# writingindy/SWMHD

Hardware: AMD Instinct MI355X
Metric: Mcell-steps/sec (fp64) on 4096^2 periodic grid (higher is better)
Workload: dtype f64

## Files before the change

swmhd_amd/csrc/common.hpp:

```cpp
#pragma once
#include <hip/hip_runtime.h>
#include <stdint.h>
#include <stdio.h>
#include <stdlib.h>
#include <type_traits>

namespace swmhd {

template <typename T>
struct OpArgs {
    const T *A;
    const T *h;
    T *Fx;
    T *Fy;
    int Nx, Ny, Hx, Hy;
    long sy;
    T dx, dy, rdx, rdy;
    int j0, j1;
    int topo_x, topo_y;
    int kernel_variant;
    int edge_cols;
};

template <typename T> hipError_t launch_lorentz_jacobian_fast(const OpArgs<T> &a, hipStream_t s);
template <typename T> hipError_t launch_lorentz_jacobian_strict(const OpArgs<T> &a, hipStream_t s);
template <typename T> hipError_t launch_lorentz_divergence_fast(const OpArgs<T> &a, hipStream_t s);
template <typename T> hipError_t launch_lorentz_divergence_strict(const OpArgs<T> &a, hipStream_t s);

template <typename T>
hipError_t launch_fill_halo_periodic(T *interior, int Nx, int Ny, int Hx, int Hy, long sy, int which, hipStream_t s);
template <typename T>
hipError_t launch_fill_halo_periodic_multi(T *const *interiors, int nfields, int Nx, int Ny, int Hx, int Hy, long sy,
                                           int which, hipStream_t s, int members = 0, long stride_m = 0);
template <typename T>
struct HaloBc {
    T *f[4];
    T grad[4][4];
    int nf, Nx, Ny, Hx, Hy, topo_x, topo_y, face_x, face_y;
    long sy;
    T dx, dy;
};
template <typename T> hipError_t launch_fill_halo_bc(const HaloBc<T> &a, hipStream_t s);
template <typename T>
struct HaloBcEns : HaloBc<T> {
    long stride_m;
    int members;
    const T *gtab;
};
template <typename T> hipError_t launch_fill_halo_bc_ensemble(const HaloBcEns<T> &a, hipStream_t s);

template <typename T>
struct TendArgs {
    const T *q1, *q2, *h, *A;
    T *G1, *G2, *Gh, *GA;
    int Nx, Ny, Hx, Hy;
    long sy;
    T dx, dy, rdx, rdy, grav, fcor;
    int j0, j1;
    int j0b, j1b;
    int fuse, first, store_G;
    int gm_prev;
    int drop_G;
    int wrap;
    int kernel_variant;
    int topo_x, topo_y;
    int leave_room;
    int edge_cols;
    T *Unew[4];
    const T *Gm[4];
    T dt, gamma, zeta;
    T dtg;
    T cu, cg;
    int anchor;
    T dtw;
};
template <typename T>
struct EnsTendArgs : TendArgs<T> {
    long stride_m;
    int members;
    int fold;
};
template <typename T, bool ENS> using TileArgs = std::conditional_t<ENS, EnsTendArgs<T>, TendArgs<T>>;
constexpr int GM_IS_PREV_STATE = 1024;
constexpr int RK3_ANCHOR = 2048;
constexpr double RK3_ANCHOR_WEIGHT = 0.25;
template <typename T>
struct Rk3Stage {
    T gamma, zeta;
    int store_G;
    const T *const *Gm;
    int flags;
};
template <typename T>
struct Rk3Buffers {
    T *cur[4], *alt[4], *gn[4], *gm[4];
    int swaps = 0;
    bool set(T *const *q, T *const *q_alt, T *const *Ga, T *const *Gb) {
        for (int f = 0; f < 4; ++f) {
            if (!q[f] || !q_alt[f] || !Ga[f] || !Gb[f]) return false;
            cur[f] = q[f]; alt[f] = q_alt[f]; gn[f] = Ga[f]; gm[f] = Gb[f];
        }
        return true;
    }
    Rk3Stage<T> stage(int st, bool anchor) const {
        const T gam[3] = {T(8.0 / 15.0), T(5.0 / 12.0), T(3.0 / 4.0)};
        const T zet[3] = {T(0), T(-17.0 / 60.0), T(-5.0 / 12.0)};
        if (anchor) return {gam[st], st == 0 ? T(RK3_ANCHOR_WEIGHT) : T(0), 0, st == 0 ? nullptr : (st == 1 ? gm : gn), RK3_ANCHOR};
        return {gam[st], zet[st], st < 2 ? 1 : 0, st == 0 ? nullptr : gm, 0};
    }
    void rotate() {
        for (int f = 0; f < 4; ++f) { T *t = cur[f]; cur[f] = alt[f]; alt[f] = t; t = gn[f]; gn[f] = gm[f]; gm[f] = t; }
        ++swaps;
    }
};

template <typename T>
struct Rk3Args {
    T *U[4];
    const T *Gn[4];
    const T *Gm[4];
    int Nx;
    long sy;
    int j0, j1;
    T dt, gamma, zeta;
    int first;
};
typedef int sw_v2i __attribute__((ext_vector_type(2)));
typedef float sw_f2 __attribute__((ext_vector_type(2)));
typedef sw_f2 sw_f2_u __attribute__((aligned(4)));
constexpr unsigned SW_OOB = 0xFFFFFFC0u;
template <typename T> __device__ __forceinline__ __amdgpu_buffer_rsrc_t out_rsrc(T *parent, unsigned bytes) {
    return __builtin_amdgcn_make_buffer_rsrc(parent, 0, (int)bytes, 0x00020000);
}
template <typename T> __device__ __forceinline__ void buffer_store(T v, __amdgpu_buffer_rsrc_t r, unsigned off) {
    if constexpr (sizeof(T) == 8) __builtin_amdgcn_raw_buffer_store_b64(__builtin_bit_cast(sw_v2i, v), r, off, 0, 0);
    else __builtin_amdgcn_raw_buffer_store_b32(__builtin_bit_cast(int, v), r, off, 0, 0);
}
template <int N> __device__ __forceinline__ void wait_vmem_all_but() {
    static_assert(N >= 0 && N < 64, "vmcnt is a 6-bit counter");
    __builtin_amdgcn_s_waitcnt((N & 15) | ((N >> 4) << 14) | (7 << 4) | (15 << 8));
}

struct ProgressPriority {
    int t1, t2, t3;
    __device__ __forceinline__ explicit ProgressPriority(int niter)
        : t1((niter * 3) / 5), t2((niter * 17) / 20), t3((niter * 19) / 20) {
        __builtin_amdgcn_s_setprio(3);
    }
    __device__ __forceinline__ void at(int it) const {
        if (it == t1) __builtin_amdgcn_s_setprio(2);
        if (it == t2) __builtin_amdgcn_s_setprio(1);
        if (it == t3) __builtin_amdgcn_s_setprio(0);
    }
};

struct MarchGeometry {
    int nt;
    int nstrips, nseg, LY;
    int wg_per_cu;
};
inline int device_cu_count() {
    static int cus = 0;
    if (cus <= 0) {
        int dev = 0, n = 0;
        if (hipGetDevice(&dev) != hipSuccess || hipDeviceGetAttribute(&n, hipDeviceAttributeMultiprocessorCount, dev) != hipSuccess || n <= 0)
            n = 256;
        cus = n;
    }
    return cus;
}
inline int env_knob(const char *name, int &cache) {
    if (cache == 0) {
        const char *e = getenv(name);
        const int v = e ? atoi(e) : 0;
        cache = v > 0 ? v : -1;
    }
    return cache > 0 ? cache : 0;
}
inline int leave_room_64ths(int rows) {
    static int cache = 0;
    const int v = env_knob("SWMHD_RING_ROOM", cache);
    return v > 0 ? (v < 32 ? v : 32) : (rows >= 3072 ? 1 : 3);
}
inline MarchGeometry march_geometry(int Nx, int rows, int xh, const int *nts, const int *wgs, int ncand, int ly_min, bool leave_room,
                                    int force_nt, int force_ly) {
    MarchGeometry g{};
    long best = -1;
    for (int k = 0; k < ncand; ++k) {
        const int txo = nts[k] - 2 * xh, ns = (Nx + txo - 1) / txo;
        const long lanes = (long)ns * nts[k];
        const bool take = force_nt ? nts[k] == force_nt : (best < 0 || lanes * 20 <= best * 19);
        if (take) { best = lanes; g.nt = nts[k]; g.nstrips = ns; g.wg_per_cu = wgs[k]; }
    }
    if (best < 0) { g.nt = nts[0]; g.nstrips = (Nx + nts[0] - 2 * xh - 1) / (nts[0] - 2 * xh); g.wg_per_cu = wgs[0]; }
    int slots = device_cu_count() * g.wg_per_cu;
    if (leave_room) slots -= (slots * leave_room_64ths(rows)) / 64;
    int LY = 32;
    for (int k = 1; k <= 64; ++k) {
        const int ns = (slots * k) / g.nstrips;
        if (ns < 1) continue;
        const int ly = (rows + ns - 1) / ns;
        if (ly <= 128) { LY = ly < ly_min ? ly_min : ly; break; }
    }
    if (force_ly > 0) LY = force_ly;
    g.LY = LY;
    g.nseg = (rows + LY - 1) / LY;
    return g;
}

template <typename T> hipError_t launch_tendency_fast(const TendArgs<T> &a, int formulation, int lorentz, hipStream_t s);
int tendency_launch_geometry(int Nx, int rows, int formulation, int elem_size, int kernel_variant, int leave_room, int wrap, int out[8]);
template <typename T> hipError_t launch_tendency_strict(const TendArgs<T> &a, int formulation, int lorentz, hipStream_t s);
template <typename T> hipError_t launch_rk3_substep_fast(const Rk3Args<T> &a, hipStream_t s);
template <typename T> hipError_t launch_tendency_ensemble_fast(const EnsTendArgs<T> &a, int formulation, int lorentz, hipStream_t s);
template <typename T> hipError_t launch_tendency_ensemble_strict(const EnsTendArgs<T> &a, int formulation, int lorentz, hipStream_t s);
template <typename T>
int tendencies_rk3_two_ranges(const T *const *q, T *const *qnew, T *const *Gn, const T *const *Gm, int Nx, int Ny, int Hx, int Hy, long sy,
                              T dx, T dy, T grav, T fcor, int formulation, int lorentz, T dt, T gamma, T zeta, int store_G, int j0, int j1,
                              int j0b, int j1b, int flags, void *stream);
template <typename T>
int fill_halo_periodic_multi(T *const *f, int nf, int Nx, int Ny, int Hx, int Hy, long sy, int which, void *stream);
template <typename T> hipError_t launch_rk3_substep_strict(const Rk3Args<T> &a, hipStream_t s);

template <typename T>
hipError_t launch_diagnostics(const T *q1, const T *q2, const T *h, const T *A, int Nx, int Ny, int j0, int j1, long sy, T dx, T dy,
                              T grav, T href, int form, double *workspace, double *out, hipStream_t s, int members = 0, long stride_m = 0);

__device__ __forceinline__ int wrap_index(int v, int n, int lo, int hi, bool wrap) {
    if (wrap) v = v < 0 ? v + n : (v >= n ? v - n : v);
    return v < lo ? lo : (v > hi ? hi : v);
}

__device__ __forceinline__ unsigned xcd_remap(unsigned bid, unsigned nblk) {
    constexpr unsigned NXCD = 8;
    unsigned q = nblk / NXCD, r = nblk % NXCD;
    unsigned x = bid % NXCD, k = bid / NXCD;
    unsigned base = x < r ? x * (q + 1) : r * (q + 1) + (x - r) * q;
    return base + k;
}

}
```

swmhd_amd/csrc/swmhd_api.hip:

```cpp
#include "../../include/swmhd.h"
#include "common.hpp"
#include <math.h>

using namespace swmhd;

namespace {

inline int hiprc(hipError_t e) { return e == hipSuccess ? SWMHD_OK : -(int)e; }

struct Ens {
    int members;
    int64_t stride_m;
    bool bc = false;
};
constexpr int ENS_FLAGS = SWMHD_STRICT | SWMHD_TILE_KERNEL | SWMHD_WRAP_X | SWMHD_WRAP_Y | SWMHD_RK3_ANCHOR;
constexpr int ENS_NOTSUP = SWMHD_BOUNDED_X | SWMHD_BOUNDED_Y | SWMHD_MARCH_KERNEL | SWMHD_GM_IS_PREV_STATE | SWMHD_LEAVE_ROOM;
constexpr int ENS_BC_FLAGS = SWMHD_STRICT | SWMHD_TILE_KERNEL | SWMHD_WRAP_X | SWMHD_WRAP_Y | SWMHD_BOUNDED_X | SWMHD_BOUNDED_Y;
constexpr int ENS_BC_NOTSUP = SWMHD_MARCH_KERNEL | SWMHD_GM_IS_PREV_STATE | SWMHD_LEAVE_ROOM | SWMHD_RK3_ANCHOR;
inline int ens_check(const Ens &e, int Ny, int Hy, int64_t sy, int flags) {
    const int ok = e.bc ? ENS_BC_FLAGS : ENS_FLAGS, notsup = e.bc ? ENS_BC_NOTSUP : ENS_NOTSUP;
    if (e.members < 1 || e.members > SWMHD_ENSEMBLE_MAX_MEMBERS) return SWMHD_EINVAL;
    if (Ny <= 0 || Hy < 0 || sy <= 0 || e.stride_m < ((int64_t)Ny + 2 * Hy) * sy) return SWMHD_EINVAL;
    if (flags & ~(ok | notsup)) return SWMHD_EINVAL;
    if (flags & notsup) return SWMHD_ENOTSUP;
// ... 93 lines not shown

template <typename T>
struct FuseRk3 {
    T *Unew[4];
    const T *const *Gm;
    T dt, gamma, zeta;
    int store_G;
};

template <typename T>
int tend_common(const T *q1, const T *q2, const T *h, const T *A, T *G1, T *G2, T *Gh, T *GA, int Nx, int Ny, int Hx, int Hy,
                int64_t sy, T dx, T dy, T grav, T fcor, int formulation, int lorentz, int j0, int j1, int flags, void *stream,
                const FuseRk3<T> *rk = nullptr, int j0b = 0, int j1b = 0, const Ens *ens = nullptr) {
    if (ens) {
        const int rc = ens_check(*ens, Ny, Hy, sy, flags);
        if (rc) return rc;
    }
    if (!q1 || !q2 || !h || !A || !G1 || !G2 || !Gh || !GA) return SWMHD_EINVAL;
    if (Nx <= 0 || Ny <= 0 || Hx < 0 || Hy < 0 || sy < (int64_t)Nx + 2 * Hx) return SWMHD_EINVAL;
    if (!(dx > T(0)) || !(dy > T(0))) return SWMHD_EINVAL;
    const int ext = ((flags & (SWMHD_WRAP_Y | SWMHD_BOUNDED_Y)) || Hy < 3) ? 0 : Hy - 3;
    if (j0 < -ext || j1 > Ny + ext || j0 > j1) return SWMHD_EINVAL;
    if (j1b > j0b && (j0b < j1 || j1b > Ny + ext)) return SWMHD_EINVAL;
    if (flags & ~(SWMHD_STRICT | SWMHD_TILE_KERNEL | SWMHD_MARCH_KERNEL | SWMHD_WRAP_X | SWMHD_WRAP_Y | SWMHD_LEAVE_ROOM | SWMHD_BOUNDED_X | SWMHD_BOUNDED_Y | SWMHD_GM_IS_PREV_STATE | SWMHD_RK3_ANCHOR)) return SWMHD_EINVAL;
    if (flags & SWMHD_GM_IS_PREV_STATE) {
        if (!rk || !rk->Gm) return SWMHD_EINVAL;
        if (flags & (SWMHD_STRICT | SWMHD_BOUNDED_X | SWMHD_BOUNDED_Y)) return SWMHD_ENOTSUP;
    }
    if (flags & SWMHD_RK3_ANCHOR) {
        if (!rk || (flags & SWMHD_GM_IS_PREV_STATE)) return SWMHD_EINVAL;
        if (flags & (SWMHD_STRICT | SWMHD_BOUNDED_X | SWMHD_BOUNDED_Y)) return SWMHD_ENOTSUP;
    }
    if (((flags & SWMHD_BOUNDED_X) && (flags & SWMHD_WRAP_X)) || ((flags & SWMHD_BOUNDED_Y) && (flags & SWMHD_WRAP_Y))) return SWMHD_EINVAL;
    if ((flags & (SWMHD_BOUNDED_X | SWMHD_BOUNDED_Y)) && (flags & SWMHD_MARCH_KERNEL)) return SWMHD_ENOTSUP;
    if (((flags & SWMHD_WRAP_X) && Hx > Nx) || ((flags & SWMHD_WRAP_Y) && Hy > Ny)) return SWMHD_EHALO;
    if (formulation != SWMHD_CONSERVATIVE && formulation != SWMHD_VECTOR_INVARIANT) return SWMHD_EINVAL;
    const bool ok = lorentz == SWMHD_LORENTZ_NONE || (formulation == SWMHD_VECTOR_INVARIANT && lorentz == SWMHD_LORENTZ_JACOBIAN) ||
                    (formulation == SWMHD_CONSERVATIVE && lorentz == SWMHD_LORENTZ_DIVERGENCE);
    if (!ok) return SWMHD_EINVAL;
    if (Hx < 3 || Hy < 3) return SWMHD_EHALO;
    if (j0 == j1 && j1b <= j0b) return SWMHD_OK;
    TendArgs<T> a;
    const long off = (long)Hy * sy + Hx;
    a.q1 = q1 + off; a.q2 = q2 + off; a.h = h + off; a.A = A + off;
    a.G1 = G1 + off; a.G2 = G2 + off; a.Gh = Gh + off; a.GA = GA + off;
    a.Nx = Nx; a.Ny = Ny; a.Hx = Hx; a.Hy = Hy; a.sy = (long)sy;
    a.dx = dx; a.dy = dy; a.rdx = T(1) / dx; a.rdy = T(1) / dy; a.grav = grav; a.fcor = fcor; a.j0 = j0; a.j1 = j1;
    a.j0b = j1b > j0b ? j0b : 0; a.j1b = j1b > j0b ? j1b : 0;
    a.fuse = 0; a.first = 0; a.store_G = 1; a.drop_G = 0; a.dt = a.gamma = a.zeta = T(0);
    a.gm_prev = (flags & SWMHD_GM_IS_PREV_STATE) ? 1 : 0; a.cu = a.cg = a.dtg = a.dtw = T(0);
    a.anchor = (flags & SWMHD_RK3_ANCHOR) ? 1 : 0;
    a.wrap = ((flags & SWMHD_WRAP_X) ? 1 : 0) | ((flags & SWMHD_WRAP_Y) ? 2 : 0);
    a.leave_room = (flags & SWMHD_LEAVE_ROOM) ? 1 : 0;
    a.edge_cols = 0;
    a.topo_x = (flags & SWMHD_BOUNDED_X) ? SWMHD_BOUNDED : SWMHD_PERIODIC; a.topo_y = (flags & SWMHD_BOUNDED_Y) ? SWMHD_BOUNDED : SWMHD_PERIODIC;
    a.kernel_variant = (flags & SWMHD_TILE_KERNEL) ? 1 : ((flags & SWMHD_MARCH_KERNEL) ? 2 : 0);
    for (int f = 0; f < 4; ++f) { a.Unew[f] = nullptr; a.Gm[f] = nullptr; }
    if (rk) {
        a.fuse = 1; a.first = rk->Gm ? 0 : 1; a.store_G = rk->store_G; a.dt = rk->dt; a.gamma = rk->gamma; a.zeta = rk->zeta;
        a.cu = a.gm_prev ? rk->zeta : T(0); a.cg = a.gm_prev ? -rk->zeta : rk->dt * rk->zeta; a.dtg = rk->dt * rk->gamma;
        if (a.anchor) {
            a.store_G = 0; a.cu = a.cg = T(0);
            a.dtw = rk->Gm ? T(0) : rk->dt * rk->zeta;
        }
        for (int f = 0; f < 4; ++f) { a.Unew[f] = rk->Unew[f] + off; a.Gm[f] = rk->Gm ? rk->Gm[f] + off : nullptr; }
    }
    hipStream_t s = (hipStream_t)stream;
    if (ens) {
        EnsTendArgs<T> e;
        static_cast<TendArgs<T> &>(e) = a;
        e.stride_m = (long)ens->stride_m; e.members = ens->members; e.fold = 1;
        return hiprc((flags & SWMHD_STRICT) ? launch_tendency_ensemble_strict<T>(e, formulation, lorentz, s)
                                            : launch_tendency_ensemble_fast<T>(e, formulation, lorentz, s));
    }
    return hiprc((flags & SWMHD_STRICT) ? launch_tendency_strict<T>(a, formulation, lorentz, s)
                                        : launch_tendency_fast<T>(a, formulation, lorentz, s));
}

template <typename T>
int tend_rk3_common(const T *const *q, T *const *qnew, T *const *Gn, const T *const *Gm, int Nx, int Ny, int Hx, int Hy, int64_t sy,
                    T dx, T dy, T grav, T fcor, int formulation, int lorentz, T dt, T gamma, T zeta, int store_G, int j0, int j1,
                    int flags, void *stream, int j0b = 0, int j1b = 0, const Ens *ens = nullptr) {
    if (ens) {
        const int rc = ens_check(*ens, Ny, Hy, sy, flags);
        if (rc) return rc;
    }
    if (!q || !qnew || !Gn) return SWMHD_EINVAL;
    for (int f = 0; f < 4; ++f) {
        if (!q[f] || !qnew[f] || !Gn[f] || (Gm && !Gm[f])) return SWMHD_EINVAL;
        for (int k = 0; k < 4; ++k)
            if (qnew[f] == q[k]) return SWMHD_EINVAL;
    }
    FuseRk3<T> rk{{qnew[0], qnew[1], qnew[2], qnew[3]}, Gm, dt, gamma, zeta, store_G ? 1 : 0};
    return tend_common<T>(q[0], q[1], q[2], q[3], Gn[0], Gn[1], Gn[2], Gn[3], Nx, Ny, Hx, Hy, sy, dx, dy, grav, fcor, formulation,
                          lorentz, j0, j1, flags, stream, &rk, j0b, j1b, ens);
}

template <typename T>
int rk3_common(T *const *U, const T *const *Gn, const T *const *Gm, int Nx, int Ny, int Hx, int Hy, int64_t sy, T dt, T gamma,
               T zeta, int j0, int j1, int flags, void *stream) {
    if (!U || !Gn || Nx <= 0 || Ny <= 0 || Hx < 0 || Hy < 0 || sy < (int64_t)Nx + 2 * Hx) return SWMHD_EINVAL;
    if (j0 < 0 || j1 > Ny || j0 > j1 || (flags & ~SWMHD_STRICT)) return SWMHD_EINVAL;
    Rk3Args<T> a;
    const long off = (long)Hy * sy + Hx;
    for (int f = 0; f < 4; ++f) {
        if (!U[f] || !Gn[f] || (Gm && !Gm[f])) return SWMHD_EINVAL;
        a.U[f] = U[f] + off; a.Gn[f] = Gn[f] + off; a.Gm[f] = Gm ? Gm[f] + off : Gn[f] + off;
// ... 233 lines not shown
```

swmhd_amd/csrc/tendency_march_kernels.inc:

```

template <typename TA> __device__ __forceinline__ void segment_rows(const TA &a, int seg, int LY, int &J0, int &J1) {
    const int nsa = (a.j1 - a.j0 + LY - 1) / LY;
    const bool second = seg >= nsa;
    const int base = second ? a.j0b + (seg - nsa) * LY : a.j0 + seg * LY, end = second ? a.j1b : a.j1;
    J0 = base;
    J1 = base + LY < end ? base + LY : end;
}

template <typename T, int LOR, int NT, int MODE>
__global__ __launch_bounds__(NT, 3) void k_tendency_vi_march(TendArgs<T> a, int nstrips, int nseg, int LY) {
    constexpr bool FUSE = (MODE & 1) != 0, HAS_GM = (MODE & 2) != 0, STORE_G = (MODE & 4) != 0, ANCHOR = (MODE & 8) != 0;
    constexpr bool STORE_W = ANCHOR && FUSE && !HAS_GM;
    constexpr int XH = 3, RW = NT + 2 * XH, TXO = NT - 2 * XH;
    __shared__ T Ru[3][RW];
    __shared__ T Rvn[1][RW];
    __shared__ __attribute__((aligned(16))) T RHA[4][RW][2];
    __shared__ T RBx[3][RW];
    __shared__ T RBy[3][RW];
    __shared__ T RFh[1][RW];
    __shared__ T RFA[1][RW];
    __shared__ T RK[1][RW];
    __shared__ T RZUV[RW][3];

    const unsigned bid = xcd_remap(blockIdx.x, (unsigned)(nstrips * nseg));
    const int strip = (int)(bid % nstrips), seg = (int)(bid / nstrips);
    const int x0 = strip * TXO;
    int J0, J1;
    segment_rows(a, seg, LY, J0, J1);
    const int c = threadIdx.x, lc = c + XH;
    const int gx = x0 - XH + c;
    const bool wx = (a.wrap & 1) != 0, wy = (a.wrap & 2) != 0;
    const int gxc = wrap_index(gx, a.Nx, -a.Hx, a.Nx + a.Hx - 1, wx);
    const int ylo = -a.Hy, yhi = a.Ny + a.Hy - 1;
    const T rdx = a.rdx, rdy = a.rdy;
    const Geo<T> g{a.dx, a.dy, a.rdx, a.rdy};
    const bool col_ok = (c >= XH) && (c < NT - XH) && (gx < a.Nx);

    T uw[8], vw[7], zw[7], svw[7], hw[7], aw[7];
    T fhy = T(0), fay = T(0), km = T(0);

    const long off0 = (long)a.Hy * a.sy + a.Hx;
    const int isy = (int)a.sy;
    auto LD = [&](const T *interior, unsigned ob) -> T { return *reinterpret_cast<const T *>(reinterpret_cast<const char *>(interior - off0) + ob); };
    const unsigned colb = (unsigned)(gxc + a.Hx) * (unsigned)sizeof(T);
    auto rowoff = [&](int row) -> unsigned { return (unsigned)((row + a.Hy) * isy) * (unsigned)sizeof(T); };
    const unsigned pbytes = (unsigned)((a.Ny + 2 * a.Hy) * isy) * (unsigned)sizeof(T);
    __amdgpu_buffer_rsrc_t rG[4], rU[4];
    if constexpr (STORE_G || STORE_W) {
        rG[0] = out_rsrc(a.G1 - off0, pbytes); rG[1] = out_rsrc(a.G2 - off0, pbytes);
        rG[2] = out_rsrc(a.Gh - off0, pbytes); rG[3] = out_rsrc(a.GA - off0, pbytes);
    }
    if constexpr (FUSE) {
#pragma unroll
        for (int f = 0; f < 4; ++f) rU[f] = out_rsrc(a.Unew[f] - off0, pbytes);
    }

    {
        const unsigned colm = (unsigned)(wrap_index(gx - 1, a.Nx, -a.Hx, a.Nx + a.Hx - 1, wx) + a.Hx) * (unsigned)sizeof(T);
        const unsigned colp = (unsigned)(wrap_index(gx + 1, a.Nx, -a.Hx, a.Nx + a.Hx - 1, wx) + a.Hx) * (unsigned)sizeof(T);
        unsigned ro[7];
#pragma unroll
        for (int k = 0; k < 7; ++k) ro[k] = rowoff(wrap_index(J0 - 3 + k, a.Ny, ylo, yhi, wy));
        T pu[7], pv[7], ph[7], pa[7], pvl[5];
#pragma unroll
        for (int k = 0; k < 7; ++k) { pu[k] = LD(a.q1, ro[k] + colb); pv[k] = LD(a.q2, ro[k] + colb); ph[k] = LD(a.h, ro[k] + colb); pa[k] = LD(a.A, ro[k] + colb); }
#pragma unroll
        for (int k = 0; k < 5; ++k) pvl[k] = LD(a.q2, ro[k + 1] + colm);
        const T ue_m = LD(a.q1, ro[2] + colp);
        T a_wm = T(0), a_em = T(0), a_wo = T(0), a_eo = T(0);
        if constexpr (LOR == 1) {
            a_wm = LD(a.A, ro[2] + colm); a_em = LD(a.A, ro[2] + colp);
            a_wo = LD(a.A, ro[3] + colm); a_eo = LD(a.A, ro[3] + colp);
        }
#pragma unroll
        for (int k = 0; k < 7; ++k) uw[k] = pu[k];
#pragma unroll
        for (int k = 0; k < 6; ++k) { vw[k] = pv[k + 1]; hw[k] = ph[k + 1]; aw[k] = pa[k + 1]; }
#pragma unroll
        for (int k = 0; k < 5; ++k) {
            zw[k] = (pv[k + 1] - pvl[k]) * rdx - (pu[k + 1] - pu[k]) * rdy;
            svw[k] = pvl[k] + pv[k + 1];
        }
        uw[7] = T(0); vw[6] = T(0); zw[5] = T(0); zw[6] = T(0); svw[5] = T(0); svw[6] = T(0); hw[6] = T(1); aw[6] = T(0);
        fhy = upwind_weno<T>(vw[2], ph);
        fay = upwind_weno<T>(vw[2], pa);
        km = T(0.25) * ((sq(uw[2]) + sq(ue_m)) + (sq(vw[1]) + sq(vw[2])));
        const int q3o = ((J0 % 3) + 3) % 3, q3m = (q3o + 2) % 3;
        Ru[q3m][lc] = uw[2];
        RHA[(J0 - 1) & 3][lc][0] = aw[1];
        RHA[J0 & 3][lc][0] = aw[2];
        if constexpr (LOR == 1) {
            const T rhm = recip<T>(hw[1]), rho = recip<T>(hw[2]);
            RBy[q3m][lc] = (T(0.5) * rdx) * (a_em - a_wm) * rhm;
            RBx[q3m][lc] = -(T(0.5) * rdy) * (aw[2] - aw[0]) * rhm;
            RBy[q3o][lc] = (T(0.5) * rdx) * (a_eo - a_wo) * rho;
            RBx[q3o][lc] = -(T(0.5) * rdy) * (aw[3] - aw[1]) * rho;
        }
    }

    auto body = [&](const int it) {
        constexpr int LU = 7, LW = 6;
        T *const U = uw, *const V = vw, *const Z = zw, *const SV = svw, *const Hh = hw, *const Aa = aw;
        const int jr = J0 - 3 + it;
        const int jo = jr - 3;
        {
            const unsigned ob = rowoff(wrap_index(jr + 1, a.Ny, ylo, yhi, wy)) + colb;
            uw[LU] = LD(a.q1, ob); vw[LW] = LD(a.q2, ob); hw[LW] = LD(a.h, ob); aw[LW] = LD(a.A, ob);
        }
        T gm0 = T(0), gm1 = T(0), gm2 = T(0), gm3 = T(0);
        const unsigned rowb = rowoff(jo);

        const int s3o = ((jo % 3) + 3) % 3, s3m = (s3o + 2) % 3, s3p = (s3o + 1) % 3;
        const int s4o = jo & 3, s4p = (jo + 1) & 3;

        Ru[s3o][lc] = U[3];
        RHA[s4o][lc][1] = Hh[2];
        RHA[s4p][lc][0] = Aa[3];
        Rvn[0][lc] = V[5];
        __syncthreads();

        {
            const T vl = Rvn[0][lc - 1];
            Z[5] = (V[5] - vl) * rdx - (U[6] - U[5]) * rdy;
            SV[5] = vl + V[5];
        }
        if constexpr (LOR == 1) {
            const T cxA = RHA[s4p][lc + 1][0] - RHA[s4p][lc - 1][0];
            const T cyA = Aa[4] - Aa[2];
            const T rh = recip<T>(Hh[3]);
            RBy[s3p][lc] = (T(0.5) * rdx) * cxA * rh;
            RBx[s3p][lc] = -(T(0.5) * rdy) * cyA * rh;
        }
        {
            const T ue2 = Ru[s3o][lc + 1];
            RK[0][lc] = T(0.25) * ((sq(U[3]) + sq(ue2)) + (sq(V[2]) + sq(V[3])));
        }
        RZUV[lc][0] = Z[2];
        RZUV[lc][1] = T(0.5) * (U[2] + U[3]);
        RZUV[lc][2] = T(0.5) * SV[2];
        {
            const T uadv = U[3];
            const bool pos = uadv >= T(0);
            const int base = pos ? lc - 3 : lc + 2, st = pos ? 1 : -1;
            T qh[5], qa[5];
#pragma unroll
            for (int k = 0; k < 5; ++k) { const T *r = RHA[s4o][base + st * k]; qa[k] = r[0]; qh[k] = r[1]; }
            RFh[0][lc] = uadv * weno5_upwind_ordered<T>(qh, pos);
            RFA[0][lc] = uadv * weno5_upwind_ordered<T>(qa, pos);
        }
        __syncthreads();
        if constexpr (FUSE && HAS_GM) {
            const unsigned og = rowb + colb;
            gm0 = LD(a.Gm[0], og); gm1 = LD(a.Gm[1], og); gm2 = LD(a.Gm[2], og); gm3 = LD(a.Gm[3], og);
        }

        const T fhy_n = upwind_weno<T>(V[3], Hh);
        const T fay_n = upwind_weno<T>(V[3], Aa);
        const T vhat = T(0.25) * (SV[2] + SV[3]);
        const T vortU = -upwind_weno_vel_raw<T>(vhat, Z, U, SV);
        const T *su0 = Ru[s3m], *su1 = Ru[s3o];
        const T ue = su1[lc + 1];
        const T uhat = T(0.25) * ((su0[lc] + su0[lc + 1]) + (U[3] + ue));
        T vortV;
        {
            const bool pos = uhat >= T(0);
            const int base = pos ? lc - 2 : lc + 3, st = pos ? 1 : -1;
            T zx[5], ufx[5], vfx[5];
#pragma unroll
            for (int k = 0; k < 5; ++k) { const T *r = RZUV[base + st * k]; zx[k] = r[0]; ufx[k] = r[1]; vfx[k] = r[2]; }
            vortV = uhat * weno5_vel_upwind_ordered<T>(zx, ufx, vfx, pos);
        }
        const T kc = RK[0][lc], kl = RK[0][lc - 1];
        const T hl = RHA[s4o][lc - 1][1];
        T Fx = T(0), Fy = T(0);
        if constexpr (LOR == 1) {
            auto A_ = [&](int di, int dj) -> T { return di == 0 ? Aa[2 + dj] : RHA[(jo + dj) & 3][lc + di][0]; };
            auto H_ = [&](int di, int dj) -> T { return di == 0 ? Hh[2 + dj] : hl; };
            auto BX_ = [&](int di, int dj) -> T { return RBx[dj < 0 ? s3m : (dj > 0 ? s3p : s3o)][lc + di]; };
            auto BY_ = [&](int di, int dj) -> T { return RBy[dj < 0 ? s3m : (dj > 0 ? s3p : s3o)][lc + di]; };
            jac_force<T>(A_, H_, BX_, BY_, 0, 0, g, Fx, Fy);
        }
        const T G1 = -vortU - (kc - kl) * rdx - a.grav * (Hh[2] - hl) * rdx + a.fcor * vhat + Fx;
        const T G2 = -vortV - (kc - km) * rdy - a.grav * (Hh[2] - Hh[1]) * rdy - a.fcor * uhat + Fy;
        const T Gh = -((RFh[0][lc + 1] - RFh[0][lc]) * rdx + (fhy_n - fhy) * rdy);
        const T GA = -((RFA[0][lc + 1] - RFA[0][lc]) * rdx + (fay_n - fay) * rdy)
                     + Aa[2] * ((ue - U[3]) * rdx + (V[3] - V[2]) * rdy);
        const unsigned o = col_ok ? rowb + colb : SW_OOB;
        const T Gs[4] = {G1, G2, Gh, GA};
        if constexpr (STORE_G) {
            const unsigned oG = a.drop_G ? SW_OOB : o;
#pragma unroll
            for (int f = 0; f < 4; ++f) buffer_store<T>(Gs[f], rG[f], oG);
        }
        if constexpr (FUSE) {
            const T Us[4] = {U[3], V[2], Hh[2], Aa[2]};
            const T Gms[4] = {gm0, gm1, gm2, gm3};
#pragma unroll
            for (int f = 0; f < 4; ++f) {
                T un;
                if constexpr (!HAS_GM) un = Us[f] + a.dtg * Gs[f];
                else if constexpr (ANCHOR) un = fma_<T>(a.dtg, Gs[f], Gms[f]);
                else if constexpr (STORE_G) un = fma_<T>(a.cg, Gms[f], fma_<T>(a.dtg, Gs[f], fma_<T>(a.cu, Us[f], Us[f])));
                else un = Us[f] + a.dt * (a.gamma * Gs[f] + a.zeta * Gms[f]);
                buffer_store<T>(un, rU[f], o);
            }
        }
        if constexpr (STORE_W) {
            const T Us[4] = {U[3], V[2], Hh[2], Aa[2]};
#pragma unroll
            for (int f = 0; f < 4; ++f) buffer_store<T>(Us[f] + a.dtw * Gs[f], rG[f], o);
        }
        fhy = fhy_n; fay = fay_n; km = kc;
        constexpr int YOUNGER = ((FUSE && HAS_GM) ? 4 : 0) + (STORE_G ? 4 : 0) + (FUSE ? 4 : 0) + (STORE_W ? 4 : 0);
        wait_vmem_all_but<YOUNGER>();
    };
    auto shift1 = [&]() {
#pragma unroll
        for (int k = 0; k < 7; ++k) uw[k] = uw[k + 1];
#pragma unroll
        for (int k = 0; k < 6; ++k) { vw[k] = vw[k + 1]; hw[k] = hw[k + 1]; aw[k] = aw[k + 1]; }
#pragma unroll
        for (int k = 0; k < 5; ++k) { zw[k] = zw[k + 1]; svw[k] = svw[k + 1]; }
    };

    const int niter = (J1 - J0) + 6;
    const ProgressPriority prio(niter);
    int it = 6;
    for (; it < niter; ++it) {
        prio.at(it);
        body(it);
        shift1();
    }
}

constexpr int CONS_W3_MODES = (1 << 7) | (1 << 5) | (1 << 4) | (1 << 9) | (1 << 11);
constexpr int cons_minwaves(int mode, int elem_size) { return elem_size == 4 ? 3 : (((CONS_W3_MODES >> mode) & 1) ? 3 : 2); }
template <typename T, int LOR, int NT, int MODE>
__global__ __launch_bounds__(NT, cons_minwaves(MODE, (int)sizeof(T))) void k_tendency_cons_march(TendArgs<T> a, int nstrips, int nseg, int LY) {
    constexpr bool FUSE = (MODE & 1) != 0, HAS_GM = (MODE & 2) != 0, STORE_G = (MODE & 4) != 0, ANCHOR = (MODE & 8) != 0;
    constexpr bool STORE_W = ANCHOR && FUSE && !HAS_GM;
    constexpr int XH = 3, RW = NT + 2 * XH, TXO = NT - 2 * XH;
    __shared__ T Ruh[3][RW];
    __shared__ T Rvh[3][RW];
    __shared__ T Rh[3][RW];
    __shared__ T RA[4][RW];
    __shared__ T RXu[1][RW];
    __shared__ T RXv[1][RW];
    __shared__ T RXa[1][RW];
    __shared__ T RUe[1][RW];
    __shared__ T RBx[1][RW];
    __shared__ T RHBx[2][RW];
    __shared__ T RBy[1][RW];
    __shared__ T RHBy[2][RW];
    __shared__ T RF1[1][RW];
    __shared__ T RG1[1][RW];

    const unsigned bid = xcd_remap(blockIdx.x, (unsigned)(nstrips * nseg));
    const int strip = (int)(bid % nstrips), seg = (int)(bid / nstrips);
    const int x0 = strip * TXO;
    int J0, J1;
    segment_rows(a, seg, LY, J0, J1);
    const int c = threadIdx.x, lc = c + XH;
    const int gx = x0 - XH + c;
    const bool wx = (a.wrap & 1) != 0, wy = (a.wrap & 2) != 0;
    const int gxc = wrap_index(gx, a.Nx, -a.Hx, a.Nx + a.Hx - 1, wx);
    const int ylo = -a.Hy, yhi = a.Ny + a.Hy - 1;
    const T rdx = a.rdx, rdy = a.rdy;
    const Geo<T> g{a.dx, a.dy, a.rdx, a.rdy};
    const bool col_ok = (c >= XH) && (c < NT - XH) && (gx < a.Nx);
    const T hg = T(0.5) * a.grav;

    T uw[6], vw[6], aw[6], hw[5];
#pragma unroll
    for (int k = 0; k < 6; ++k) { uw[k] = T(0); vw[k] = T(0); aw[k] = T(0); }
#pragma unroll
    for (int k = 0; k < 5; ++k) hw[k] = T(1);
    T bxw[5], byw[5], hbx_pub = T(0), hby_pub = T(0);
#pragma unroll
// ... 254 lines not shown
```

swmhd_amd/csrc/tendency_tile_kernels.inc:

```

#ifndef SWMHD_STRICT
#error "include with SWMHD_STRICT defined"
#endif

namespace swmhd {
namespace {

constexpr bool STRICT = (SWMHD_STRICT != 0);

#include <type_traits>
#include "tile_common.inc"
#include "lorentz_device.inc"
#include "sw_device.inc"

template <typename T>
__device__ __forceinline__ unsigned ens_member(EnsTendArgs<T> &a, unsigned ntiles) {
    unsigned m, t;
    if (a.fold) {
        const unsigned L = xcd_remap(blockIdx.x, ntiles * (unsigned)a.members);
        m = L / ntiles; t = L - m * ntiles;
    } else {
        m = blockIdx.y; t = xcd_remap(blockIdx.x, ntiles);
    }
    const long o = (long)m * a.stride_m;
// ... 231 lines not shown
                        un = Us[f] + (a.dt * a.gamma) * Gs[f] + a.zeta * (Us[f] - a.Gm[f][o]);
                    } else {
                        un = Us[f] + a.dt * (a.gamma * Gs[f] + a.zeta * a.Gm[f][o]);
                    }
                    a.Unew[f][o] = un;
                }
            }
        }
    }
}

template <typename T>
__global__ void k_rk3_substep(Rk3Args<T> a) {
    const int x = blockIdx.x * blockDim.x + threadIdx.x;
    const int y = a.j0 + blockIdx.y;
    if (x >= a.Nx || y >= a.j1) return;
    const long o = (long)y * a.sy + x;
#pragma unroll
    for (int f = 0; f < 4; ++f) {
        T u = a.U[f][o];
        if (a.first) {
            if constexpr (STRICT) u += a.dt * a.gamma * a.Gn[f][o];
            else u += (a.dt * a.gamma) * a.Gn[f][o];
        } else {
            u += a.dt * (a.gamma * a.Gn[f][o] + a.zeta * a.Gm[f][o]);
        }
        a.U[f][o] = u;
    }
}

#if !SWMHD_STRICT
#include "tendency_march_kernels.inc"
#include "tendency_pk_kernels.inc"
#endif

}

#define LAUNCH_NAME_(base, sfx) base##sfx
#define LAUNCH_NAME(base, sfx) LAUNCH_NAME_(base, sfx)

constexpr long SW_MARCH_MIN_CELLS = 330000L;

#if !SWMHD_STRICT
static bool tendency_uses_packed_fp32(int Nx, int formulation, int wrap) {
    return formulation == 1 && (wrap & 1) && (Nx % 2 == 0) && Nx >= 8;
}
static MarchGeometry packed_fp32_geometry(int Nx, int rows, int leave_room) {
    static int ly_cache = 0;
    static const int cols[1] = {512}, wgs[1] = {3};
    MarchGeometry g = march_geometry(Nx, rows, 4, cols, wgs, 1, 6, leave_room != 0, 0, env_knob("SWMHD_T_LY", ly_cache));
    g.nt = 256;
    return g;
}
static MarchGeometry tendency_march_geometry(int Nx, int rows, int formulation, int leave_room, int elem_size, int mode = 7) {
    static int ly_cache = 0, nt_cache = 0;
    const int force_ly = env_knob("SWMHD_T_LY", ly_cache), force_nt = env_knob("SWMHD_T_NT", nt_cache);
    if (formulation == 1) {
        static const int nts[2] = {256, 128}, wgs64[2] = {3, 6}, wgs32[2] = {4, 8};
        return march_geometry(Nx, rows, 3, nts, elem_size == 8 ? wgs64 : wgs32, 2, 6, leave_room != 0, force_nt, force_ly);
    }
    const int w = cons_minwaves(mode, elem_size);
    const int nts[2] = {256, 128}, wgs[2] = {w, 2 * w};
    return march_geometry(Nx, rows, 3, nts, wgs, 2, 6, leave_room != 0, force_nt, force_ly);
}
template <typename T> static int march_stage_mode(TendArgs<T> &a, int formulation) {
    int mode = (a.fuse ? 1 : 0) | ((a.fuse && !a.first) ? 2 : 0) | ((a.store_G || !a.fuse) ? 4 : 0) | (a.anchor ? 8 : 0);
    const bool cons64 = formulation == 0 && sizeof(T) == 8;
    if (mode == 3 && (a.gm_prev || (cons64 && cons_minwaves(7, 8) > cons_minwaves(3, 8)))) { mode = 7; a.drop_G = 1; }
    if (mode == 1 && cons64 && cons_minwaves(5, 8) > cons_minwaves(1, 8)) { mode = 5; a.drop_G = 1; }
    return mode;
}
template <typename T> using MarchKernel = void (*)(TendArgs<T>, int, int, int);
template <typename T, int MODE> static MarchKernel<T> march_kernel(int formulation, int lorentz, int nt, bool packed) {
    if constexpr (std::is_same<T, float>::value) {
        if (packed) return lorentz == 1 ? k_tendency_vi_march_pk<1, 256, MODE> : k_tendency_vi_march_pk<0, 256, MODE>;
    }
    if (formulation == 1) {
        if (nt == 128) return lorentz == 1 ? k_tendency_vi_march<T, 1, 128, MODE> : k_tendency_vi_march<T, 0, 128, MODE>;
        return lorentz == 1 ? k_tendency_vi_march<T, 1, 256, MODE> : k_tendency_vi_march<T, 0, 256, MODE>;
    }
    if (nt == 128) return lorentz == 2 ? k_tendency_cons_march<T, 2, 128, MODE> : k_tendency_cons_march<T, 0, 128, MODE>;
    return lorentz == 2 ? k_tendency_cons_march<T, 2, 256, MODE> : k_tendency_cons_march<T, 0, 256, MODE>;
}
template <typename T> static MarchKernel<T> march_kernel(int mode, int formulation, int lorentz, int nt, bool packed) {
    switch (mode) {
    case 1: return march_kernel<T, 1>(formulation, lorentz, nt, packed);
    case 3: return march_kernel<T, 3>(formulation, lorentz, nt, packed);
    case 4: return march_kernel<T, 4>(formulation, lorentz, nt, packed);
    case 5: return march_kernel<T, 5>(formulation, lorentz, nt, packed);
    case 7: return march_kernel<T, 7>(formulation, lorentz, nt, packed);
    case 9: return march_kernel<T, 9>(formulation, lorentz, nt, packed);
    case 11: return march_kernel<T, 11>(formulation, lorentz, nt, packed);
    default: return nullptr;
    }
}
#endif

template <typename T, int RY, bool BND = false, bool ENS = false>
static hipError_t launch_tile(const TileArgs<T, ENS> &a, int formulation, int lorentz, int ntx, int nty, hipStream_t s) {
    constexpr int TX = 64, TYB = 4;
    dim3 grid(ntx * nty);
    const dim3 block(TX, TYB);
    if constexpr (ENS) grid = a.fold ? dim3(ntx * nty * a.members) : dim3(ntx * nty, a.members);
    if (formulation == 1 && lorentz == 1) hipLaunchKernelGGL((k_tendency_tile<T, 1, 1, TX, TYB, RY, BND, ENS>), grid, block, 0, s, a, ntx, nty);
    else if (formulation == 1 && lorentz == 0) hipLaunchKernelGGL((k_tendency_tile<T, 1, 0, TX, TYB, RY, BND, ENS>), grid, block, 0, s, a, ntx, nty);
    else if (formulation == 0 && lorentz == 2) hipLaunchKernelGGL((k_tendency_tile<T, 0, 2, TX, TYB, RY, BND, ENS>), grid, block, 0, s, a, ntx, nty);
    else if (formulation == 0 && lorentz == 0) hipLaunchKernelGGL((k_tendency_tile<T, 0, 0, TX, TYB, RY, BND, ENS>), grid, block, 0, s, a, ntx, nty);
    else return hipErrorInvalidValue;
    return hipGetLastError();
}

template <typename T>
hipError_t LAUNCH_NAME(launch_tendency_, LAUNCH_SFX)(const TendArgs<T> &a, int formulation, int lorentz, hipStream_t s) {
    constexpr int TX = 64, TYB = 4, RY = 2;
    const bool two = a.j1b > a.j0b;
    const int rows_b = two ? a.j1b - a.j0b : 0;
    [[maybe_unused]] const int rows = a.j1 - a.j0 + rows_b;
    auto one_by_one = [&]() {
        TendArgs<T> b = a;
        b.j0b = b.j1b = 0;
        hipError_t e = LAUNCH_NAME(launch_tendency_, LAUNCH_SFX)<T>(b, formulation, lorentz, s);
        if (e != hipSuccess) return e;
        b.j0 = a.j0b; b.j1 = a.j1b;
        return LAUNCH_NAME(launch_tendency_, LAUNCH_SFX)<T>(b, formulation, lorentz, s);
    };
    if (two && a.j1 <= a.j0) return one_by_one();
    int ntx = (a.Nx + TX - 1) / TX, nty = (a.j1 - a.j0 + TYB * RY - 1) / (TYB * RY) + (rows_b + TYB * RY - 1) / (TYB * RY);
    if (ntx <= 0 || nty <= 0) return hipSuccess;
    if (a.edge_cols) {
        const int ne = (a.Nx % TX == 0 || a.Nx % TX >= 8) ? 2 : 3;
        ntx = ntx < ne ? ntx : ne;
    }
#if !SWMHD_STRICT
    const bool fits32 = (long)(a.Ny + 2 * a.Hy) * a.sy * (long)sizeof(T) < (1L << 32) - 64;
    const bool bnd = a.topo_x == 1 || a.topo_y == 1;
    const bool march = !bnd && fits32 && (a.kernel_variant == 2 || (a.kernel_variant == 0 && (long)a.Nx * rows >= SW_MARCH_MIN_CELLS));
    if (bnd && !two && !a.edge_cols && fits32 && a.kernel_variant == 0 && (long)a.Nx * rows >= SW_MARCH_MIN_CELLS && a.Nx >= 4 * TX &&
        a.Ny >= 48) {
        constexpr int FW = 8;
        TendArgs<T> p = a;
        p.topo_x = p.topo_y = 0;
        hipError_t e = LAUNCH_NAME(launch_tendency_, LAUNCH_SFX)<T>(p, formulation, lorentz, s);
        if (e != hipSuccess) return e;
        TendArgs<T> f = a;
        f.kernel_variant = 1;
        if (a.topo_y == 1) {
            const int a0 = a.j0, a1 = a.j1 < FW ? a.j1 : FW, b0 = a.j0 > a.Ny - FW ? a.j0 : a.Ny - FW, b1 = a.j1;
            f.j0 = a0; f.j1 = a1 > a0 ? a1 : a0; f.j0b = b0; f.j1b = b1 > b0 ? b1 : b0;
            if (f.j1 > f.j0 || f.j1b > f.j0b) {
                e = LAUNCH_NAME(launch_tendency_, LAUNCH_SFX)<T>(f, formulation, lorentz, s);
                if (e != hipSuccess) return e;
            }
        }
        if (a.topo_x == 1) {
            f.j0 = a.j0; f.j1 = a.j1; f.j0b = f.j1b = 0; f.edge_cols = 1;
            e = LAUNCH_NAME(launch_tendency_, LAUNCH_SFX)<T>(f, formulation, lorentz, s);
            if (e != hipSuccess) return e;
        }
        return hipSuccess;
    }
    auto two_range_segments = [&](int LY) { return (a.j1 - a.j0 + LY - 1) / LY + (rows_b + LY - 1) / LY; };
    if (march) {
        TendArgs<T> ax = a;
        const int mode = march_stage_mode(ax, formulation);
        const bool packed = sizeof(T) == 4 && tendency_uses_packed_fp32(a.Nx, formulation, a.wrap);
        const MarchGeometry mg = packed ? packed_fp32_geometry(a.Nx, rows, a.leave_room)
                                        : tendency_march_geometry(a.Nx, rows, formulation, a.leave_room, (int)sizeof(T), mode);
        const int nstrips = mg.nstrips, LY = mg.LY, nseg = two ? two_range_segments(LY) : mg.nseg;
        const MarchKernel<T> k = march_kernel<T>(mode, formulation, lorentz, mg.nt, packed);
        if (!k) return hipErrorInvalidValue;
        hipLaunchKernelGGL(k, dim3(nstrips * nseg), dim3(mg.nt), 0, s, ax, nstrips, nseg, LY);
        return hipGetLastError();
    }
#endif
#if !SWMHD_STRICT
    if (!(a.topo_x == 1 || a.topo_y == 1) && (long)a.Nx * rows < SW_MARCH_MIN_CELLS) {
        constexpr int RY1 = 1;
        const int nty1 = (a.j1 - a.j0 + TYB * RY1 - 1) / (TYB * RY1) + (rows_b + TYB * RY1 - 1) / (TYB * RY1);
        return launch_tile<T, RY1>(a, formulation, lorentz, ntx, nty1, s);
    }
#endif
    if (a.topo_x == 1 || a.topo_y == 1) return launch_tile<T, RY, true>(a, formulation, lorentz, ntx, nty, s);
    return launch_tile<T, RY>(a, formulation, lorentz, ntx, nty, s);
}

template <typename T>
hipError_t LAUNCH_NAME(launch_tendency_ensemble_, LAUNCH_SFX)(const EnsTendArgs<T> &a, int formulation, int lorentz, hipStream_t s) {
    constexpr int TX = 64, TYB = 4;
    static int ry_cache = 0, map_cache = 0;
    const int rows = a.j1 - a.j0;
    if (rows <= 0 || a.members <= 0) return hipSuccess;
    const bool bnd = a.topo_x == 1 || a.topo_y == 1;
    const int force_ry = bnd ? 0 : env_knob("SWMHD_ENS_RY", ry_cache), map = env_knob("SWMHD_ENS_MAP", map_cache);
    const int ry = bnd ? 2 : (force_ry == 1 || force_ry == 2 ? force_ry : ((!STRICT && (long)a.Nx * rows < SW_MARCH_MIN_CELLS) ? 1 : 2));
    const int ntx = (a.Nx + TX - 1) / TX, nty = (rows + TYB * ry - 1) / (TYB * ry);
    const long blocks = (long)ntx * nty * a.members;
    if (blocks >= (1L << 31) || (map == 2 && a.members > 65535)) return hipErrorInvalidConfiguration;
    EnsTendArgs<T> e = a;
    e.fold = map == 2 ? 0 : 1;
    if (bnd) return launch_tile<T, 2, true, true>(e, formulation, lorentz, ntx, nty, s);
    return ry == 1 ? launch_tile<T, 1, false, true>(e, formulation, lorentz, ntx, nty, s)
                   : launch_tile<T, 2, false, true>(e, formulation, lorentz, ntx, nty, s);
}

template <typename T>
hipError_t LAUNCH_NAME(launch_rk3_substep_, LAUNCH_SFX)(const Rk3Args<T> &a, hipStream_t s) {
    if (a.j1 <= a.j0) return hipSuccess;
    hipLaunchKernelGGL((k_rk3_substep<T>), dim3((a.Nx + 255) / 256, a.j1 - a.j0), dim3(256), 0, s, a);
    return hipGetLastError();
}

#if !SWMHD_STRICT
int tendency_launch_geometry(int Nx, int rows, int formulation, int elem_size, int kernel_variant, int leave_room, int wrap, int out[8]) {
    const bool march = (kernel_variant == 2 || (kernel_variant == 0 && (long)Nx * rows >= SW_MARCH_MIN_CELLS));
    if (march && elem_size == 4 && tendency_uses_packed_fp32(Nx, formulation, wrap)) {
        const MarchGeometry mg = packed_fp32_geometry(Nx, rows, leave_room);
        out[0] = 3; out[1] = mg.nt; out[2] = mg.nstrips; out[3] = mg.nseg; out[4] = mg.LY; out[5] = mg.wg_per_cu; out[6] = 2;
    } else if (march) {
        const MarchGeometry mg = tendency_march_geometry(Nx, rows, formulation, leave_room, elem_size);
        out[0] = 2; out[1] = mg.nt; out[2] = mg.nstrips; out[3] = mg.nseg; out[4] = mg.LY; out[5] = mg.wg_per_cu; out[6] = 3;
    } else {
        const int ry = (kernel_variant == 1 || (long)Nx * rows >= SW_MARCH_MIN_CELLS) ? 2 : 1;
        out[0] = 1; out[1] = 256; out[2] = (Nx + 63) / 64; out[3] = (rows + 4 * ry - 1) / (4 * ry); out[4] = 4 * ry; out[5] = 0; out[6] = 3;
    }
// ... 14 lines not shown
```

Measured before the change: 14010.

## Fold narrow last march strip into half-workgroups covering two segments

When the last x-strip of the vector-invariant fp64 march kernel covers at most half a 256-thread workgroup, one workgroup now processes two row segments of that strip, each with half its threads. The aim is to avoid launching mostly-idle workgroups for the remainder strip, and the segment count is rebalanced over half-strip units. Shared-memory row buffers grow to hold two half-width tiles, and rows past a half's end are masked with out-of-bounds offsets. The cost is extra index arithmetic, more LDS use, and possible imbalance when the two halves have different row counts.

```diff
diff --git a/swmhd_amd/csrc/common.hpp b/swmhd_amd/csrc/common.hpp
--- a/swmhd_amd/csrc/common.hpp
+++ b/swmhd_amd/csrc/common.hpp
@@ -66,6 +66,7 @@
     int topo_x, topo_y;
     int leave_room;
     int edge_cols;
+    int fold_last;
     T *Unew[4];
     const T *Gm[4];
     T dt, gamma, zeta;
@@ -158,6 +159,8 @@
     int nt;
     int nstrips, nseg, LY;
     int wg_per_cu;
+    int fold;
+    int blocks() const { return fold ? (nstrips - 1) * nseg + (nseg + 1) / 2 : nstrips * nseg; }
 };
 inline int device_cu_count() {
     static int cus = 0;
@@ -183,7 +186,7 @@
     return v > 0 ? (v < 32 ? v : 32) : (rows >= 3072 ? 1 : 3);
 }
 inline MarchGeometry march_geometry(int Nx, int rows, int xh, const int *nts, const int *wgs, int ncand, int ly_min, bool leave_room,
-                                    int force_nt, int force_ly) {
+                                    int force_nt, int force_ly, int fold_nt = 0) {
     MarchGeometry g{};
     long best = -1;
     for (int k = 0; k < ncand; ++k) {
@@ -193,11 +196,13 @@
         if (take) { best = lanes; g.nt = nts[k]; g.nstrips = ns; g.wg_per_cu = wgs[k]; }
     }
     if (best < 0) { g.nt = nts[0]; g.nstrips = (Nx + nts[0] - 2 * xh - 1) / (nts[0] - 2 * xh); g.wg_per_cu = wgs[0]; }
+    g.fold = fold_nt && g.nt == fold_nt && g.nstrips > 1 && Nx - (g.nstrips - 1) * (g.nt - 2 * xh) <= g.nt / 2 - 2 * xh ? 1 : 0;
+    const int halves = 2 * g.nstrips - g.fold;
     int slots = device_cu_count() * g.wg_per_cu;
     if (leave_room) slots -= (slots * leave_room_64ths(rows)) / 64;
     int LY = 32;
     for (int k = 1; k <= 64; ++k) {
-        const int ns = (slots * k) / g.nstrips;
+        const int ns = (2 * slots * k) / halves;
         if (ns < 1) continue;
         const int ly = (rows + ns - 1) / ns;
         if (ly <= 128) { LY = ly < ly_min ? ly_min : ly; break; }
diff --git a/swmhd_amd/csrc/swmhd_api.hip b/swmhd_amd/csrc/swmhd_api.hip
--- a/swmhd_amd/csrc/swmhd_api.hip
+++ b/swmhd_amd/csrc/swmhd_api.hip
@@ -169,7 +169,7 @@
     a.anchor = (flags & SWMHD_RK3_ANCHOR) ? 1 : 0;
     a.wrap = ((flags & SWMHD_WRAP_X) ? 1 : 0) | ((flags & SWMHD_WRAP_Y) ? 2 : 0);
     a.leave_room = (flags & SWMHD_LEAVE_ROOM) ? 1 : 0;
-    a.edge_cols = 0;
+    a.edge_cols = 0; a.fold_last = 0;
     a.topo_x = (flags & SWMHD_BOUNDED_X) ? SWMHD_BOUNDED : SWMHD_PERIODIC; a.topo_y = (flags & SWMHD_BOUNDED_Y) ? SWMHD_BOUNDED : SWMHD_PERIODIC;
     a.kernel_variant = (flags & SWMHD_TILE_KERNEL) ? 1 : ((flags & SWMHD_MARCH_KERNEL) ? 2 : 0);
     for (int f = 0; f < 4; ++f) { a.Unew[f] = nullptr; a.Gm[f] = nullptr; }
diff --git a/swmhd_amd/csrc/tendency_march_kernels.inc b/swmhd_amd/csrc/tendency_march_kernels.inc
--- a/swmhd_amd/csrc/tendency_march_kernels.inc
+++ b/swmhd_amd/csrc/tendency_march_kernels.inc
@@ -11,7 +11,9 @@
 __global__ __launch_bounds__(NT, 3) void k_tendency_vi_march(TendArgs<T> a, int nstrips, int nseg, int LY) {
     constexpr bool FUSE = (MODE & 1) != 0, HAS_GM = (MODE & 2) != 0, STORE_G = (MODE & 4) != 0, ANCHOR = (MODE & 8) != 0;
     constexpr bool STORE_W = ANCHOR && FUSE && !HAS_GM;
-    constexpr int XH = 3, RW = NT + 2 * XH, TXO = NT - 2 * XH;
+    constexpr bool FOLDS = NT == 256 && sizeof(T) == 8;
+    constexpr int XH = 3, NH = NT / 2, TXO = NT - 2 * XH;
+    constexpr int RW = FOLDS ? 2 * (NH + 2 * XH) : NT + 2 * XH;
     __shared__ T Ru[3][RW];
     __shared__ T Rvn[1][RW];
     __shared__ __attribute__((aligned(16))) T RHA[4][RW][2];
@@ -22,19 +24,35 @@
     __shared__ T RK[1][RW];
     __shared__ T RZUV[RW][3];
 
-    const unsigned bid = xcd_remap(blockIdx.x, (unsigned)(nstrips * nseg));
-    const int strip = (int)(bid % nstrips), seg = (int)(bid / nstrips);
+    const bool fold = FOLDS && a.fold_last;
+    const int nfull = fold ? nstrips - 1 : nstrips;
+    const unsigned bid = xcd_remap(blockIdx.x, (unsigned)(fold ? nfull * nseg + (nseg + 1) / 2 : nstrips * nseg));
+    int strip = (int)(bid % nstrips), seg = (int)(bid / nstrips);
+    bool half_wg = false;
+    int hf = 0;
+    if (fold) {
+        const int pr = (int)bid / (2 * nfull + 1), r = (int)bid - pr * (2 * nfull + 1);
+        half_wg = r >= (2 * pr + 1 < nseg ? 2 : 1) * nfull;
+        if (half_wg) hf = __builtin_amdgcn_readfirstlane((int)threadIdx.x / NH);
+        strip = half_wg ? nfull : r % nfull;
+        seg = 2 * pr + (half_wg ? hf : r / nfull);
+    }
+    int J0, J1, niter;
+    segment_rows(a, seg - hf, LY, J0, J1);
+    niter = (J1 - J0) + 6;
+    if (hf) {
+        if (seg < nseg) segment_rows(a, seg, LY, J0, J1);
+        else J0 = J1 = a.j1;
+    }
     const int x0 = strip * TXO;
-    int J0, J1;
-    segment_rows(a, seg, LY, J0, J1);
-    const int c = threadIdx.x, lc = c + XH;
+    const int c = threadIdx.x - hf * NH, lc = c + XH + hf * (NH + 2 * XH);
     const int gx = x0 - XH + c;
     const bool wx = (a.wrap & 1) != 0, wy = (a.wrap & 2) != 0;
     const int gxc = wrap_index(gx, a.Nx, -a.Hx, a.Nx + a.Hx - 1, wx);
     const int ylo = -a.Hy, yhi = a.Ny + a.Hy - 1;
     const T rdx = a.rdx, rdy = a.rdy;
     const Geo<T> g{a.dx, a.dy, a.rdx, a.rdy};
-    const bool col_ok = (c >= XH) && (c < NT - XH) && (gx < a.Nx);
+    const bool col_ok = (c >= XH) && (c < (half_wg ? NH : NT) - XH) && (gx < a.Nx);
 
     T uw[8], vw[7], zw[7], svw[7], hw[7], aw[7];
     T fhy = T(0), fay = T(0), km = T(0);
@@ -45,6 +63,7 @@
     const unsigned colb = (unsigned)(gxc + a.Hx) * (unsigned)sizeof(T);
     auto rowoff = [&](int row) -> unsigned { return (unsigned)((row + a.Hy) * isy) * (unsigned)sizeof(T); };
     const unsigned pbytes = (unsigned)((a.Ny + 2 * a.Hy) * isy) * (unsigned)sizeof(T);
+    const unsigned rowlast = rowoff(J1 - 1);
     __amdgpu_buffer_rsrc_t rG[4], rU[4];
     if constexpr (STORE_G || STORE_W) {
         rG[0] = out_rsrc(a.G1 - off0, pbytes); rG[1] = out_rsrc(a.G2 - off0, pbytes);
@@ -108,7 +127,9 @@
             uw[LU] = LD(a.q1, ob); vw[LW] = LD(a.q2, ob); hw[LW] = LD(a.h, ob); aw[LW] = LD(a.A, ob);
         }
         T gm0 = T(0), gm1 = T(0), gm2 = T(0), gm3 = T(0);
-        const unsigned rowb = rowoff(jo);
+        const bool live = jo < J1;
+        const unsigned rowb = live ? rowoff(jo) : pbytes;
+        const unsigned og = (live ? rowb : rowlast) + colb;
 
         const int s3o = ((jo % 3) + 3) % 3, s3m = (s3o + 2) % 3, s3p = (s3o + 1) % 3;
         const int s4o = jo & 3, s4p = (jo + 1) & 3;
@@ -150,7 +171,6 @@
         }
         __syncthreads();
         if constexpr (FUSE && HAS_GM) {
-            const unsigned og = rowb + colb;
             gm0 = LD(a.Gm[0], og); gm1 = LD(a.Gm[1], og); gm2 = LD(a.Gm[2], og); gm3 = LD(a.Gm[3], og);
         }
 
@@ -185,7 +205,7 @@
         const T Gh = -((RFh[0][lc + 1] - RFh[0][lc]) * rdx + (fhy_n - fhy) * rdy);
         const T GA = -((RFA[0][lc + 1] - RFA[0][lc]) * rdx + (fay_n - fay) * rdy)
                      + Aa[2] * ((ue - U[3]) * rdx + (V[3] - V[2]) * rdy);
-        const unsigned o = col_ok ? rowb + colb : SW_OOB;
+        const unsigned o = FUSE && HAS_GM ? (col_ok && live ? og : SW_OOB) : (col_ok ? rowb + colb : SW_OOB);
         const T Gs[4] = {G1, G2, Gh, GA};
         if constexpr (STORE_G) {
             const unsigned oG = a.drop_G ? SW_OOB : o;
@@ -223,7 +243,6 @@
         for (int k = 0; k < 5; ++k) { zw[k] = zw[k + 1]; svw[k] = svw[k + 1]; }
     };
 
-    const int niter = (J1 - J0) + 6;
     const ProgressPriority prio(niter);
     int it = 6;
     for (; it < niter; ++it) {
diff --git a/swmhd_amd/csrc/tendency_tile_kernels.inc b/swmhd_amd/csrc/tendency_tile_kernels.inc
--- a/swmhd_amd/csrc/tendency_tile_kernels.inc
+++ b/swmhd_amd/csrc/tendency_tile_kernels.inc
@@ -307,12 +307,18 @@
     g.nt = 256;
     return g;
 }
-static MarchGeometry tendency_march_geometry(int Nx, int rows, int formulation, int leave_room, int elem_size, int mode = 7) {
+static bool tendency_fold_enabled() {
+    static const bool on = [] { const char *e = getenv("SWMHD_T_FOLD"); return !e || atoi(e) != 0; }();
+    return on;
+}
+static MarchGeometry tendency_march_geometry(int Nx, int rows, int formulation, int leave_room, int elem_size, int mode = 7,
+                                             bool fold_ok = true) {
     static int ly_cache = 0, nt_cache = 0;
     const int force_ly = env_knob("SWMHD_T_LY", ly_cache), force_nt = env_knob("SWMHD_T_NT", nt_cache);
     if (formulation == 1) {
         static const int nts[2] = {256, 128}, wgs64[2] = {3, 6}, wgs32[2] = {4, 8};
-        return march_geometry(Nx, rows, 3, nts, elem_size == 8 ? wgs64 : wgs32, 2, 6, leave_room != 0, force_nt, force_ly);
+        const int fold_nt = elem_size == 8 && fold_ok && tendency_fold_enabled() ? 256 : 0;
+        return march_geometry(Nx, rows, 3, nts, elem_size == 8 ? wgs64 : wgs32, 2, 6, leave_room != 0, force_nt, force_ly, fold_nt);
     }
     const int w = cons_minwaves(mode, elem_size);
     const int nts[2] = {256, 128}, wgs[2] = {w, 2 * w};
@@ -419,12 +425,14 @@
         TendArgs<T> ax = a;
         const int mode = march_stage_mode(ax, formulation);
         const bool packed = sizeof(T) == 4 && tendency_uses_packed_fp32(a.Nx, formulation, a.wrap);
-        const MarchGeometry mg = packed ? packed_fp32_geometry(a.Nx, rows, a.leave_room)
-                                        : tendency_march_geometry(a.Nx, rows, formulation, a.leave_room, (int)sizeof(T), mode);
-        const int nstrips = mg.nstrips, LY = mg.LY, nseg = two ? two_range_segments(LY) : mg.nseg;
+        const bool fold_ok = !two && (long)(a.Ny + 2 * a.Hy + 1) * a.sy * (long)sizeof(T) < (1L << 32) - 64;
+        MarchGeometry mg = packed ? packed_fp32_geometry(a.Nx, rows, a.leave_room)
+                                  : tendency_march_geometry(a.Nx, rows, formulation, a.leave_room, (int)sizeof(T), mode, fold_ok);
+        if (two) mg.nseg = two_range_segments(mg.LY);
+        ax.fold_last = mg.fold;
         const MarchKernel<T> k = march_kernel<T>(mode, formulation, lorentz, mg.nt, packed);
         if (!k) return hipErrorInvalidValue;
-        hipLaunchKernelGGL(k, dim3(nstrips * nseg), dim3(mg.nt), 0, s, ax, nstrips, nseg, LY);
+        hipLaunchKernelGGL(k, dim3(mg.blocks()), dim3(mg.nt), 0, s, ax, mg.nstrips, mg.nseg, mg.LY);
         return hipGetLastError();
     }
 #endif
```

Measured after the change: 14240 (median of 6 runs). +1.6%, better.
